# ParsaEsmati/SEA

Measured on AMD Instinct MI355X. Metric: rollout steps/sec (full-context forward, recompute mode) on cylinder_flow-shaped fields, higher is better.
Workload: dtype bf16

## Files before the change

### sea_amd/build.py

```python
from __future__ import annotations

import os
import subprocess
import sys
from concurrent.futures import ThreadPoolExecutor

HERE = os.path.dirname(os.path.abspath(__file__))
CSRC = os.path.join(HERE, "csrc")
BUILD = os.path.join(CSRC, "build")
LIB = os.path.join(CSRC, "libsea_hip.so")
SOURCES = ["core.hip", "gemm.hip", "gemm_norm.hip", "mlp_fused.hip", "attention.hip", "rowops.hip", "train.hip", "bwd.hip", "attention_bwd.hip", "kvstep.hip", "gemv.hip", "chain.hip", "gemm_adaln.hip", "mlp_block.hip", "adaln_qkv.hip", "gemm256.hip", "gemm_ws.hip", "encoder_block.hip", "decode_loss.hip", "ensemble.hip"]
HEADERS = ["sea_common.hpp", "gemm_core.hpp", "norm_epilogue.hpp", "gemm_tile.hpp", os.path.join("..", "..", "include", "sea_hip.h")]
FLAGS = (os.environ.get("SEA_EXTRA_FLAGS", "").split()) + ["--offload-arch=gfx950", "-O3", "-std=c++17", "-fPIC", "-mcode-object-version=5", "-mllvm", "-amdgpu-mfma-vgpr-form=1", "-ffast-math", "-fno-finite-math-only", "-fgpu-flush-denormals-to-zero", "-Wall", "-Wno-unused-function", "-Wno-unused-result"]


FILE_FLAGS: dict = {}

_PK_SRC1_HI = __import__("re").compile(r"^\s*v_pk_(?:fma|mul|add)_f32\b.*\bop_sel:\[[01],1[,\]]")


def lint_isa(asm_path: str) -> list:
    bad, kernel = [], "?"
    with open(asm_path) as f:
        for no, line in enumerate(f, 1):
            if line[:1].isalpha() or line[:1] == "_":
                kernel = line.split(":")[0]
            elif _PK_SRC1_HI.match(line):
                bad.append((kernel, no, line.strip()))
    return bad


def _hipcc() -> str:
    for cand in (os.environ.get("HIPCC"), "/opt/rocm/bin/hipcc", "hipcc"):
        if cand and (os.path.isabs(cand) and os.path.exists(cand) or not os.path.isabs(cand)):
            return cand
    raise RuntimeError("hipcc not found")


def _asm_of(obj: str) -> str:
    return obj[:-2] + "-hip-amdgcn-amd-amdhsa-gfx950.s"


def _stale(target: str, deps) -> bool:
    if not os.path.exists(target):
        return True
    t = os.path.getmtime(target)
    return any(os.path.getmtime(d) > t for d in deps if os.path.exists(d))


def build(force: bool = False, verbose: bool = True) -> str:
    import fcntl

    os.makedirs(BUILD, exist_ok=True)
    with open(os.path.join(CSRC, ".build.lock"), "w") as lock:
        fcntl.flock(lock, fcntl.LOCK_EX)
        try:
            return _build_locked(force, verbose)
        finally:
            fcntl.flock(lock, fcntl.LOCK_UN)


def _build_locked(force: bool, verbose: bool) -> str:
    hipcc = _hipcc()
    srcs = [s for s in SOURCES if os.path.exists(os.path.join(CSRC, s))]
    hdrs = [os.path.join(CSRC, h) for h in HEADERS]
    objs = []
    jobs = []
    os.makedirs(BUILD, exist_ok=True)
    for s in srcs:
        src = os.path.join(CSRC, s)
        obj = os.path.join(BUILD, s.replace(".hip", ".o"))
        objs.append(obj)
        if force or _stale(obj, [src] + hdrs) or not os.path.exists(_asm_of(obj)):
            jobs.append([hipcc] + FLAGS + FILE_FLAGS.get(s, []) + ["-save-temps=obj", "-c", src, "-o", obj])

    def run(cmd):
        if verbose:
            print(" ".join(cmd), flush=True)
        r = subprocess.run(cmd, stdout=subprocess.PIPE, stderr=subprocess.STDOUT, text=True)
        return r.returncode, r.stdout

    if jobs:
        with ThreadPoolExecutor(max_workers=min(4, len(jobs))) as ex:
            for rc, out in ex.map(run, jobs):
                if out.strip() and verbose:
                    print(out)
                if rc != 0:
                    raise RuntimeError("hipcc failed:\n" + out)
    for f in os.listdir(BUILD):
        stem = f.split("-hip-")[0].split(".")[0]
        if (not (f.endswith(".o") and "-hip-" not in f) and not f.endswith("-hip-amdgcn-amd-amdhsa-gfx950.s")) or stem + ".hip" not in srcs:
            try:
                os.remove(os.path.join(BUILD, f))
            except FileNotFoundError:
                pass
    findings = []
    for obj in objs:
        for kernel, no, ins in lint_isa(_asm_of(obj)):
            findings.append(f"{os.path.basename(_asm_of(obj))}:{no}: {kernel}: {ins}")
    if findings:
        for obj in objs:
            if lint_isa(_asm_of(obj)):
                os.remove(obj)
        raise RuntimeError("sea_amd.build: packed fp32 instructions with the low half reading the high dword of src1 (gfx950 erratum, see build.py):\n  "
                           + "\n  ".join(findings[:40]) + (f"\n  ... {len(findings) - 40} more" if len(findings) > 40 else ""))
    if force or jobs or _stale(LIB, objs):
        rc, out = run([hipcc, "--offload-arch=gfx950", "-shared", "-fPIC", "-o", LIB] + objs)
        if rc != 0:
            raise RuntimeError("link failed:\n" + out)
    return LIB


if __name__ == "__main__":
    print(build(force="--force" in sys.argv))
```

### sea_amd/csrc/mlp_block.hip

```cpp
#include "gemm_core.hpp"
#include <stdlib.h>

struct MlpBlockLaunch {
    SeaMlpGroup g1[SEA_MAX_MLP_GROUPS];
    SeaMlp2Group g2[SEA_MAX_MLP_GROUPS];
    int tile_start[SEA_MAX_MLP_GROUPS + 1];
    int xcd_start[SEA_MAX_MLP_GROUPS + 1];
    int n_groups;
    float eps;
    int per_xcd;
    int probe;
};

__device__ __forceinline__ void glds16_blk(const void* gsrc, unsigned lds_addr) {
    unsigned keep;
    asm volatile("s_mov_b32 %0, m0\n\ts_mov_b32 m0, %2\n\ts_nop 0\n\tglobal_load_lds_dwordx4 %1, off\n\ts_mov_b32 m0, %0"
                 : "=&s"(keep) : "v"(gsrc), "s"(lds_addr) : "memory");
}

__device__ __forceinline__ void glds16_blk_s(const void* ubase, unsigned lane_off, unsigned lds_addr) {
    unsigned keep;
    asm volatile("s_mov_b32 %0, m0\n\ts_mov_b32 m0, %3\n\ts_nop 0\n\tglobal_load_lds_dwordx4 %1, %2\n\ts_mov_b32 m0, %0"
                 : "=&s"(keep) : "v"(lane_off), "s"(ubase), "s"(lds_addr) : "memory");
}

template <int KT, int NSB>
struct MlpBlockCfg {
    static constexpr int BM = 32, BKB = 128, NS = 4, NW = 8;
    static constexpr int E = KT * 64, S = NSB * 128;
    static constexpr int A_BYTES = KT * BM * BKB, STAGE = KT * 64 * BKB;
    static constexpr int PRM_OFF = A_BYTES + NS * STAGE;
    static constexpr int P1_BYTES = PRM_OFF + 2 * S * 4;
    static constexpr int SLAB_PITCH = 128 * 4 + 16, SLAB = BM * SLAB_PITCH;
    static constexpr int X3_OFF = NW * SLAB;
    static constexpr int RED2_OFF = X3_OFF + KT * BM * BKB;
    static constexpr int P2_BYTES = RED2_OFF + 2 * NW * BM * 4;
    static constexpr int RS = KT == 4 ? 8 : 4, SLOT = 16 * 128;
    static constexpr int RING_OFF = KT == 4 ? A_BYTES : P1_BYTES;
    static constexpr int RING_END = RING_OFF + NW * RS * SLOT;
    static constexpr int BYTES_ = P1_BYTES > P2_BYTES ? P1_BYTES : P2_BYTES;
    static constexpr int BYTES = BYTES_ > RING_END ? BYTES_ : RING_END;
};

__device__ __forceinline__ f32x4 mma16_first(const uint4& a, const uint4& b) {
    return __builtin_amdgcn_mfma_f32_16x16x32_bf16(__builtin_bit_cast(bf16x8, a), __builtin_bit_cast(bf16x8, b), f32x4{0.f, 0.f, 0.f, 0.f}, 0, 0, 0);
}

__device__ __forceinline__ constexpr int blk_col_base(int t, int half, int wq) { return (t >> 1) * 512 + half * 256 + wq * 64 + (t & 1) * 32; }

template <int KT, int NSB>
__global__ __launch_bounds__(512) void mlp_block_kernel(const MlpBlockLaunch L) {
    using T = __bf16;
    using Cf = MlpBlockCfg<KT, NSB>;
    constexpr int BM = 32, BKB = 128, BK = 64, NS = 4, NW = 8;
    constexpr int E = Cf::E, S = Cf::S, NSTAGE = S / 64, NT = NSB / 2;
    constexpr int A_BYTES = Cf::A_BYTES, STAGE = Cf::STAGE;
    constexpr int LPS = KT * 8 / NW;
    constexpr int PRM_OFF = Cf::PRM_OFF;
    constexpr int B1_OFF = 0, RED_OFF = S * 4;
    static_assert(RED_OFF + 2 * NW * BM * 4 <= A_BYTES && (S / 256) * 1024 <= A_BYTES && LPS * NW == KT * 8 && NT % 2 == 0 && Cf::BYTES <= 160 * 1024, "LDS layout of sea_mlp_block");
    static_assert((NT / 2) * 512 == S, "blk_col_base covers the hidden columns once");
    extern __shared__ __attribute__((aligned(16))) char smem[];
    int tile, gi = 0;
    if (L.per_xcd < 0) {
        const int xcd = (int)(blockIdx.x & 7), idx = (int)(blockIdx.x >> 3);
        if (xcd >= L.xcd_start[L.n_groups]) return;
        while (gi + 1 < L.n_groups && xcd >= L.xcd_start[gi + 1]) ++gi;
        tile = L.tile_start[gi] + (xcd - L.xcd_start[gi]) * 32 + idx;
        if (tile >= L.tile_start[gi + 1]) return;
    } else {
        tile = L.per_xcd > 0 ? (int)(blockIdx.x & 7) * L.per_xcd + (int)(blockIdx.x >> 3) : (int)blockIdx.x;
        if (tile >= L.tile_start[L.n_groups]) return;
        while (gi + 1 < L.n_groups && tile >= L.tile_start[gi + 1]) ++gi;
    }
    const SeaMlpGroup& G = L.g1[gi];
    const SeaMlp2Group& H = L.g2[gi];
    const int m0 = (tile - L.tile_start[gi]) * BM, M = G.M;
    const int tid = threadIdx.x, lane = tid & 63;
    const int wave = __builtin_amdgcn_readfirstlane(tid >> 6);
    const int r = lane & 15, g = lane >> 4;
    const int half = wave >> 2, wq = wave & 3;
    const T* A = static_cast<const T*>(G.A);
    const T* W = static_cast<const T*>(G.W1);
    const unsigned lds_base = __builtin_amdgcn_readfirstlane((unsigned)(uintptr_t)smem);
    const int rl = lane >> 3;
    const int chunk = (lane & 7) ^ (rl & 7);
    for (int p = wave; p < 2 * (S / 256); p += NW) {
        const float* src = p < S / 256 ? G.lnw : G.lnb;
        const int q = p < S / 256 ? p : p - S / 256;
        glds16_blk(src + q * 256 + lane * 4, lds_base + (unsigned)(PRM_OFF + p * 1024));
    }
    for (int p = wave; G.X32 == nullptr && p < KT * (BM / 8); p += NW) {
        const int kt = p / (BM / 8), u = p - kt * (BM / 8);
        int row = m0 + u * 8 + rl;
        row = row < M ? row : M - 1;
        glds16_blk(A + (int64_t)row * G.lda + kt * BK + chunk * 8, lds_base + (unsigned)(kt * BM * BKB + u * 8 * BKB));
    }
    const unsigned w1_lane = (unsigned)(((8 * (rl >> 2) + (rl & 3)) * G.ldw + chunk * 8) * 2);
    auto dma_stage = [&](int s) {
        const unsigned base = lds_base + (unsigned)(A_BYTES + (s % NS) * STAGE);
        const int t = s >> 2, u = (s >> 1) & 1, hs = s & 1;
#pragma unroll
        for (int i = 0; i < LPS; ++i) {
            const int p = i * NW + wave;
            const int kt = p >> 3, u8 = p & 7;
            const int urow = blk_col_base(t, hs, u8 >> 1) + 16 * (u8 & 1) + 4 * u;
            glds16_blk_s(W + (int64_t)urow * G.ldw + kt * BK, w1_lane, base + (unsigned)(kt * 64 * BKB + u8 * 8 * BKB));
        }
    };
    dma_stage(0);
    if (G.X32 != nullptr) {
        constexpr int CPT = E / 16;
        const int prow = tid >> 4, pl = tid & 15;
        int row = m0 + prow;
        row = row < M ? row : M - 1;
        const int c0 = pl * CPT;
        float xv[CPT];
#pragma unroll
        for (int c = 0; c < CPT; c += 4) load4(G.X32 + (int64_t)row * G.ldx32 + c0 + c, *reinterpret_cast<float(*)[4]>(xv + c));
        if (G.addend != nullptr) {
#pragma unroll
            for (int c = 0; c < CPT; c += 4) {
                float av[4];
                load4(G.addend + (int64_t)row * G.ldadd + c0 + c, av);
#pragma unroll
                for (int e = 0; e < 4; ++e) xv[c + e] += av[e];
            }
        }
        float gq[CPT], bq[CPT];
#pragma unroll
        for (int c = 0; c < CPT; c += 4) {
            load4(G.gamma + c0 + c, *reinterpret_cast<float(*)[4]>(gq + c));
#pragma unroll
            for (int e = 0; e < 4; ++e) bq[c + e] = 0.f;
            if (G.beta != nullptr) load4(G.beta + c0 + c, *reinterpret_cast<float(*)[4]>(bq + c));
            if (G.mod != nullptr) {
                float mw[4], mb[4];
                const T* mod = static_cast<const T*>(G.mod) + (int64_t)row * G.ldmod;
                load4(mod + c0 + c, mw);
                load4(mod + E + c0 + c, mb);
#pragma unroll
                for (int e = 0; e < 4; ++e) {
                    gq[c + e] += 1.0f + mw[e];
                    bq[c + e] += mb[e];
                }
            }
        }
        float s4[4] = {0.f, 0.f, 0.f, 0.f};
#pragma unroll
        for (int c = 0; c < CPT; c += 4)
#pragma unroll
            for (int e = 0; e < 4; ++e) s4[e] = add1(s4[e], xv[c + e]);
        float sm_ = add1(add1(s4[0], s4[1]), add1(s4[2], s4[3]));
#pragma unroll
        for (int o = 8; o >= 1; o >>= 1) sm_ += __shfl_xor(sm_, o);
        const float mean = sm_ * (1.0f / (float)E);
        float q4[4] = {0.f, 0.f, 0.f, 0.f};
#pragma unroll
        for (int c = 0; c < CPT; c += 4)
#pragma unroll
            for (int e = 0; e < 4; ++e) {
                const float d_ = xv[c + e] - mean;
                q4[e] = fma1(d_, d_, q4[e]);
            }
        float sq = add1(add1(q4[0], q4[1]), add1(q4[2], q4[3]));
#pragma unroll
        for (int o = 8; o >= 1; o >>= 1) sq += __shfl_xor(sq, o);
        const float rstd = 1.0f / sqrtf(sq * (1.0f / (float)E) + G.norm_eps);
#pragma unroll
        for (int c = 0; c < CPT; c += 8) {
            const int col = c0 + c, kt = col >> 6, ck = (col & 63) >> 3;
            bf16x8 pv;
#pragma unroll
            for (int e = 0; e < 8; ++e) pv[e] = (__bf16)((xv[c + e] - mean) * rstd * gq[c + e] + bq[c + e]);
            *reinterpret_cast<bf16x8*>(smem + kt * BM * BKB + prow * BKB + ((ck ^ (prow & 7)) << 4)) = pv;
        }
        asm volatile("s_waitcnt vmcnt(0) lgkmcnt(0)" ::: "memory");
    }
    for (int s = 1; s < NS - 1; ++s) dma_stage(s);

    const T* W2 = static_cast<const T*>(H.W2);
    const unsigned w2_lane = (unsigned)((rl * H.ldw2 + chunk * 8) * 2);
    const T* Wp = static_cast<const T*>(H.Wproj);
    const unsigned wp_lane = (unsigned)((rl * H.ldwp + chunk * 8) * 2);
    constexpr int NSLOT = (E / 16) * (NT / 2);
    constexpr int NJ = E / NW / 16;
    constexpr int NX = NJ * KT;
    auto w2_slot = [&](int k) {
        const unsigned dst = lds_base + (unsigned)(Cf::RING_OFF + (wave * Cf::RS + (k % Cf::RS)) * Cf::SLOT);
        if (k < NSLOT) {
            const int tau = k / (E / 16), j = k - tau * (E / 16);
            const T* ub = W2 + (int64_t)(j * 16) * H.ldw2 + blk_col_base(2 * tau, half, wq);
#pragma unroll
            for (int u = 0; u < 2; ++u)
                glds16_blk_s(ub + (int64_t)(8 * u) * H.ldw2, w2_lane, dst + (unsigned)(u * 1024));
        } else {
            const int kk = k - NSLOT, j = kk / KT, kt = kk - j * KT;
            const T* ub = Wp + (int64_t)(wave * (E / NW) + j * 16) * H.ldwp + kt * BK;
#pragma unroll
            for (int u = 0; u < 2; ++u)
                glds16_blk_s(ub + (int64_t)(8 * u) * H.ldwp, wp_lane, dst + (unsigned)(u * 1024));
        }
    };
    uint4 hid[NT][2];
    float mean[2], rstd[2];
    {
        f32x4 acc[NSB][2];
        uint4 areg[KT][2][2];
#pragma unroll
        for (int i = 0; i < NSB; ++i) {
            acc[i][0] = f32x4{0.f, 0.f, 0.f, 0.f};
            acc[i][1] = f32x4{0.f, 0.f, 0.f, 0.f};
        }
#pragma unroll
        for (int s = 0; s < NSTAGE; ++s) {
            if (s + 2 < NSTAGE) asm volatile("s_waitcnt vmcnt(%0) lgkmcnt(0)" ::"n"(2 * LPS) : "memory");
            else if (s + 1 < NSTAGE) asm volatile("s_waitcnt vmcnt(%0) lgkmcnt(0)" ::"n"(LPS) : "memory");
            else asm volatile("s_waitcnt vmcnt(0) lgkmcnt(0)" ::: "memory");
            __builtin_amdgcn_s_barrier();
            if (s + NS - 1 < NSTAGE) dma_stage(s + NS - 1);
            if (s == 0) {
                const char* sA = smem + r * BKB;
#pragma unroll
                for (int kt = 0; kt < KT; ++kt)
#pragma unroll
                    for (int kc = 0; kc < 2; ++kc) {
                        const int off = ((kc * 4 + g) ^ (r & 7)) << 4;
                        areg[kt][kc][0] = *reinterpret_cast<const uint4*>(sA + kt * BM * BKB + off);
                        areg[kt][kc][1] = *reinterpret_cast<const uint4*>(sA + kt * BM * BKB + 16 * BKB + off);
                    }
                asm volatile("s_waitcnt lgkmcnt(0)" ::: "memory");
            }
            if (s == 1)
                for (int p = wave; p < S / 256; p += NW) glds16_blk(G.b1 + p * 256 + lane * 4, lds_base + (unsigned)(B1_OFF + p * 1024));
            if ((s & 1) == half) {
                const char* sW = smem + A_BYTES + (s % NS) * STAGE + (wq * 16 + r) * BKB;
#pragma unroll
                for (int kt = 0; kt < KT; ++kt)
#pragma unroll
                    for (int kc = 0; kc < 2; ++kc) {
                        const int off = ((kc * 4 + g) ^ (r & 7)) << 4;
                        const uint4 wf = *reinterpret_cast<const uint4*>(sW + kt * 64 * BKB + off);
                        mma16<T>(wf, areg[kt][kc][0], acc[s >> 1][0]);
                        mma16<T>(wf, areg[kt][kc][1], acc[s >> 1][1]);
                    }
            }
        }
        if (L.probe == 1) return;
        float* red = reinterpret_cast<float*>(smem + RED_OFF);
        const float* pb1 = reinterpret_cast<const float*>(smem + B1_OFF);
        const float* pgm = reinterpret_cast<const float*>(smem + PRM_OFF);
        const float* pbt = pgm + S;
        const float inv_s = 1.0f / (float)S;
        float sum[2] = {0.f, 0.f};
#pragma unroll
        for (int i = 0; i < NSB; ++i) {
            const int n = blk_col_base(i >> 1, half, wq) + 8 * g + 4 * (i & 1);
            float bv[4];
            load4(pb1 + n, bv);
#pragma unroll
            for (int mb = 0; mb < 2; ++mb) {
#pragma unroll
                for (int q = 0; q < 4; ++q) acc[i][mb][q] += bv[q];
                sum[mb] += (acc[i][mb][0] + acc[i][mb][1]) + (acc[i][mb][2] + acc[i][mb][3]);
            }
        }
#pragma unroll
        for (int mb = 0; mb < 2; ++mb) {
            sum[mb] += __shfl_xor(sum[mb], 16);
            sum[mb] += __shfl_xor(sum[mb], 32);
            if (g == 0) red[wave * 32 + mb * 16 + r] = sum[mb];
        }
        __syncthreads();
#pragma unroll
        for (int k = 0; k < Cf::RS - 1; ++k) w2_slot(k);
        float sq[2] = {0.f, 0.f};
#pragma unroll
        for (int mb = 0; mb < 2; ++mb) {
            float t = 0.f;
#pragma unroll
            for (int w = 0; w < NW; ++w) t += red[w * 32 + mb * 16 + r];
            mean[mb] = t * inv_s;
        }
#pragma unroll
        for (int i = 0; i < NSB; ++i)
#pragma unroll
            for (int mb = 0; mb < 2; ++mb)
#pragma unroll
                for (int q = 0; q < 4; ++q) {
                    const float c = acc[i][mb][q] - mean[mb];
                    sq[mb] += c * c;
                }
#pragma unroll
        for (int mb = 0; mb < 2; ++mb) {
            sq[mb] += __shfl_xor(sq[mb], 16);
            sq[mb] += __shfl_xor(sq[mb], 32);
            if (g == 0) red[256 + wave * 32 + mb * 16 + r] = sq[mb];
        }
        asm volatile("s_waitcnt lgkmcnt(0)" ::: "memory");
        __builtin_amdgcn_s_barrier();
#pragma unroll
        for (int mb = 0; mb < 2; ++mb) {
            float t = 0.f;
#pragma unroll
            for (int w = 0; w < NW; ++w) t += red[256 + w * 32 + mb * 16 + r];
            rstd[mb] = 1.0f / sqrtf(t * inv_s + L.eps);
        }
#pragma unroll
        for (int i = 0; i < NSB; ++i) {
            const int n = blk_col_base(i >> 1, half, wq) + 8 * g + 4 * (i & 1);
            float gm[4], bt[4];
            load4(pgm + n, gm);
            load4(pbt + n, bt);
#pragma unroll
            for (int mb = 0; mb < 2; ++mb) {
                bf16x4 y;
#pragma unroll
                for (int q = 0; q < 4; ++q) y[q] = (__bf16)gelu_erf_bf16((acc[i][mb][q] - mean[mb]) * rstd[mb] * gm[q] + bt[q]);
                uint2 y2 = *reinterpret_cast<const uint2*>(&y);
                asm volatile("" : "+v"(y2.x), "+v"(y2.y));
                if (i & 1) {
                    hid[i >> 1][mb].z = y2.x;
                    hid[i >> 1][mb].w = y2.y;
                } else {
                    hid[i >> 1][mb].x = y2.x;
                    hid[i >> 1][mb].y = y2.y;
                }
            }
            __builtin_amdgcn_sched_barrier(0);
        }
    }
    __builtin_amdgcn_sched_barrier(0);
    if (L.probe == 2) {
        asm volatile("s_waitcnt vmcnt(0)" ::: "memory");
        return;
    }

    constexpr int NJB = E / 16;
    constexpr int NTOT = NSLOT + NX;
    f32x4 acc2[2][NJB];
    uint4 wp[KT * 2][NJ];
#pragma unroll
    for (int k = 0; k < NTOT; ++k) {
        const int tau = k / NJB, j = k - tau * NJB;
        {
            constexpr int AFTER_MAX = Cf::RS - 2;
            const int after = NTOT - 1 - k < AFTER_MAX ? NTOT - 1 - k : AFTER_MAX;
            switch (after) {
                case 6: asm volatile("s_waitcnt vmcnt(12) lgkmcnt(0)" ::: "memory"); break;
                case 5: asm volatile("s_waitcnt vmcnt(10) lgkmcnt(0)" ::: "memory"); break;
                case 4: asm volatile("s_waitcnt vmcnt(8) lgkmcnt(0)" ::: "memory"); break;
                case 3: asm volatile("s_waitcnt vmcnt(6) lgkmcnt(0)" ::: "memory"); break;
                case 2: asm volatile("s_waitcnt vmcnt(4) lgkmcnt(0)" ::: "memory"); break;
                case 1: asm volatile("s_waitcnt vmcnt(2) lgkmcnt(0)" ::: "memory"); break;
                default: asm volatile("s_waitcnt vmcnt(0) lgkmcnt(0)" ::: "memory"); break;
            }
        }
        if (k + Cf::RS - 1 < NTOT) w2_slot(k + Cf::RS - 1);
        const char* sl = smem + Cf::RING_OFF + (wave * Cf::RS + (k % Cf::RS)) * Cf::SLOT + r * 128;
        if (k >= NSLOT) {
            const int kk = k - NSLOT, jp = kk / KT, kt = kk - jp * KT;
#pragma unroll
            for (int kc = 0; kc < 2; ++kc) wp[kt * 2 + kc][jp] = *reinterpret_cast<const uint4*>(sl + (((kc * 4 + g) ^ (r & 7)) << 4));
            continue;
        }
#pragma unroll
        for (int u2 = 0; u2 < 2; ++u2) {
            const uint4 w = *reinterpret_cast<const uint4*>(sl + (((u2 * 4 + g) ^ (r & 7)) << 4));
            const int t = 2 * tau + u2;
            if (t == 0) {
                acc2[0][j] = mma16_first(w, hid[0][0]);
                acc2[1][j] = mma16_first(w, hid[0][1]);
            } else {
                mma16<T>(w, hid[t][0], acc2[0][j]);
                mma16<T>(w, hid[t][1], acc2[1][j]);
            }
        }
        __builtin_amdgcn_sched_barrier(0);
    }
    __syncthreads();
    if (L.probe == 3) return;
    {
    int tid_l = threadIdx.x;
    asm volatile("" : "+v"(tid_l));
    const int tid = tid_l, lane = tid & 63, r = lane & 15, g = lane >> 4;
    (void)lane;
    constexpr int NH = E / 128, JH = 8;
    const int srow = tid >> 4, scb = (tid & 15) * 8;
    float resv[NH][8];
    {
        int row = m0 + srow;
        row = row < M ? row : M - 1;
#pragma unroll
        for (int h = 0; h < NH; ++h) {
            const int col = h * 128 + scb;
            float b2a[4], b2b[4];
            load4(H.b2 + col, b2a);
            load4(H.b2 + col + 4, b2b);
            float ra[4], rb[4];
            if (H.R != nullptr) {
                load4(H.R + (int64_t)row * H.ldr + col, ra);
                load4(H.R + (int64_t)row * H.ldr + col + 4, rb);
            } else {
                load4(G.X32 + (int64_t)row * G.ldx32 + col, ra);
                load4(G.X32 + (int64_t)row * G.ldx32 + col + 4, rb);
                if (G.addend != nullptr) {
                    float aa[4], ab[4];
                    load4(G.addend + (int64_t)row * G.ldadd + col, aa);
                    load4(G.addend + (int64_t)row * G.ldadd + col + 4, ab);
#pragma unroll
                    for (int q = 0; q < 4; ++q) {
                        ra[q] += aa[q];
                        rb[q] += ab[q];
                    }
                }
            }
#pragma unroll
            for (int q = 0; q < 4; ++q) {
                resv[h][q] = b2a[q] + ra[q];
                resv[h][4 + q] = b2b[q] + rb[q];
            }
        }
    }
    constexpr int CPT = E / 16;
    const int ec0 = (tid & 15) * CPT;
    float ebp[CPT], egq[CPT], ebq[CPT];
    const bool has_norm = H.gamma != nullptr;
#pragma unroll
    for (int h = 0; h < NH; ++h) {
        char* slab = smem + wave * Cf::SLAB;
#pragma unroll
        for (int mb = 0; mb < 2; ++mb)
#pragma unroll
            for (int j = 0; j < JH; ++j)
                *reinterpret_cast<f32x4*>(slab + (mb * 16 + r) * Cf::SLAB_PITCH + (j * 16 + g * 4) * 4) = acc2[mb][h * JH + j];
        if (h == NH - 1) {
            __builtin_amdgcn_sched_barrier(0);
            int m = m0 + srow;
            m = m < M ? m : M - 1;
#pragma unroll
            for (int c = 0; c < CPT; c += 4) {
                load4(H.bproj + ec0 + c, *reinterpret_cast<float(*)[4]>(ebp + c));
#pragma unroll
                for (int q = 0; q < 4; ++q) egq[c + q] = ebq[c + q] = 0.f;
                if (has_norm) {
                    load4(H.gamma + ec0 + c, *reinterpret_cast<float(*)[4]>(egq + c));
                    if (H.beta != nullptr) load4(H.beta + ec0 + c, *reinterpret_cast<float(*)[4]>(ebq + c));
                    if (H.mod != nullptr) {
                        float mw[4], mb[4];
                        const T* mod = static_cast<const T*>(H.mod) + (int64_t)m * H.ldmod;
                        load4(mod + ec0 + c, mw);
                        load4(mod + E + ec0 + c, mb);
#pragma unroll
                        for (int q = 0; q < 4; ++q) {
                            egq[c + q] += 1.0f + mw[q];
                            ebq[c + q] += mb[q];
                        }
                    }
                }
            }
        }
        asm volatile("s_waitcnt lgkmcnt(0)" ::: "memory");
        __builtin_amdgcn_s_barrier();
        {
            float v[8];
#pragma unroll
            for (int q = 0; q < 8; ++q) v[q] = resv[h][q];
#pragma unroll
            for (int w = 0; w < NW; ++w) {
                const float4 a = *reinterpret_cast<const float4*>(smem + w * Cf::SLAB + srow * Cf::SLAB_PITCH + scb * 4);
                const float4 b = *reinterpret_cast<const float4*>(smem + w * Cf::SLAB + srow * Cf::SLAB_PITCH + scb * 4 + 16);
                v[0] += a.x; v[1] += a.y; v[2] += a.z; v[3] += a.w;
                v[4] += b.x; v[5] += b.y; v[6] += b.z; v[7] += b.w;
            }
            const int col = h * 128 + scb, kt = col >> 6, ck = (col & 63) >> 3;
            bf16x8 pv;
#pragma unroll
            for (int q = 0; q < 8; ++q) pv[q] = (__bf16)v[q];
            *reinterpret_cast<bf16x8*>(smem + Cf::X3_OFF + kt * BM * BKB + srow * BKB + ((ck ^ (srow & 7)) << 4)) = pv;
        }
        asm volatile("s_waitcnt lgkmcnt(0)" ::: "memory");
        __builtin_amdgcn_s_barrier();
        if (L.probe == 5 + h) return;
    }

    if (L.probe == 4) return;
    f32x4 acc3[2][NJ];
    {
        const char* sA = smem + Cf::X3_OFF + r * BKB;
#pragma unroll
        for (int kt = 0; kt < KT; ++kt)
#pragma unroll
            for (int kc = 0; kc < 2; ++kc) {
                const int off = ((kc * 4 + g) ^ (r & 7)) << 4;
                const uint4 af0 = *reinterpret_cast<const uint4*>(sA + kt * BM * BKB + off);
                const uint4 af1 = *reinterpret_cast<const uint4*>(sA + kt * BM * BKB + 16 * BKB + off);
#pragma unroll
                for (int j = 0; j < NJ; ++j) {
                    if (kt == 0 && kc == 0) {
                        acc3[0][j] = mma16_first(wp[0][j], af0);
                        acc3[1][j] = mma16_first(wp[0][j], af1);
                    } else {
                        mma16<T>(wp[kt * 2 + kc][j], af0, acc3[0][j]);
                        mma16<T>(wp[kt * 2 + kc][j], af1, acc3[1][j]);
                    }
                }
            }
    }
    constexpr int SEG = 80, YP = (E / 16) * SEG + 16;
    static_assert(BM * YP <= Cf::X3_OFF, "the y tile lies in front of the x3 tile");
#pragma unroll
    for (int i = 0; i < 2; ++i)
#pragma unroll
        for (int j = 0; j < NJ; ++j) {
            const int n = wave * (E / NW) + j * 16 + g * 4;
            *reinterpret_cast<f32x4*>(smem + (i * 16 + r) * YP + (n >> 4) * SEG + (n & 15) * 4) = acc3[i][j];
        }
    asm volatile("s_waitcnt lgkmcnt(0)" ::: "memory");
    __builtin_amdgcn_s_barrier();
    {
        float v[CPT];
#pragma unroll
        for (int c = 0; c < CPT; c += 4) {
            const float4 y = *reinterpret_cast<const float4*>(smem + srow * YP + ((ec0 + c) >> 4) * SEG + ((ec0 + c) & 15) * 4);
            v[c] = y.x + ebp[c]; v[c + 1] = y.y + ebp[c + 1]; v[c + 2] = y.z + ebp[c + 2]; v[c + 3] = y.w + ebp[c + 3];
        }
        if (has_norm) {
            float s4[4] = {0.f, 0.f, 0.f, 0.f};
#pragma unroll
            for (int c = 0; c < CPT; c += 4)
#pragma unroll
                for (int e = 0; e < 4; ++e) s4[e] = add1(s4[e], v[c + e]);
            float sm_ = add1(add1(s4[0], s4[1]), add1(s4[2], s4[3]));
#pragma unroll
            for (int o = 8; o >= 1; o >>= 1) sm_ += __shfl_xor(sm_, o);
            const float mean2 = sm_ * (1.0f / (float)E);
            float q4[4] = {0.f, 0.f, 0.f, 0.f};
#pragma unroll
            for (int c = 0; c < CPT; c += 4)
#pragma unroll
                for (int e = 0; e < 4; ++e) {
                    const float d_ = v[c + e] - mean2;
                    q4[e] = fma1(d_, d_, q4[e]);
                }
            float sq = add1(add1(q4[0], q4[1]), add1(q4[2], q4[3]));
#pragma unroll
            for (int o = 8; o >= 1; o >>= 1) sq += __shfl_xor(sq, o);
            const float rstd2 = 1.0f / sqrtf(sq * (1.0f / (float)E) + L.eps);
#pragma unroll
            for (int c = 0; c < CPT; ++c) v[c] = (v[c] - mean2) * rstd2 * egq[c] + ebq[c];
        }
        const int m = m0 + srow;
        if (m < M) {
#pragma unroll
            for (int c = 0; c < CPT; c += 4) {
                if (H.Y32 != nullptr) store4(H.Y32 + (int64_t)m * H.ldy32 + ec0 + c, v[c], v[c + 1], v[c + 2], v[c + 3]);
                if (H.Yact != nullptr) store4(static_cast<T*>(H.Yact) + (int64_t)m * H.ldyact + ec0 + c, v[c], v[c + 1], v[c + 2], v[c + 3]);
            }
        }
    }
    }
}

extern "C" int sea_mlp_block(const SeaMlpGroup* g1, const SeaMlp2Group* g2, int n_groups, float eps, int dtype, void* stream) {
    SEA_REQUIRE(g1 != nullptr && g2 != nullptr && n_groups >= 1 && n_groups <= SEA_MAX_MLP_GROUPS, "sea_mlp_block: n_groups=%d out of range", n_groups);
    const int E = g1[0].E, S = g1[0].S;
    const bool shape_ok = (E == 256 && S == 2048) || (E == 128 && S == 1024);
    if (dtype != SEA_BF16 || !shape_ok) {
        sea_set_error("sea_mlp_block: unsupported dtype / shape (dtype=%d E=%d S=%d): bf16, (E, S) in {(256, 2048), (128, 1024)}", dtype, E, S);
        return SEA_EUNSUPPORTED;
    }
    MlpBlockLaunch L;
    memset(&L, 0, sizeof(L));
    int total = 0;
    for (int i = 0; i < n_groups; ++i) {
        const SeaMlpGroup& G = g1[i];
        const SeaMlp2Group& H = g2[i];
        SEA_REQUIRE(G.E == E && G.S == S && H.E == E && H.S == S && G.M >= 1 && H.M == G.M, "sea_mlp_block[%d]: the groups of a launch share E and S; both halves the same M", i);
        SEA_REQUIRE((G.A || G.X32) && G.W1 && G.b1 && G.lnw && G.lnb, "sea_mlp_block[%d]: null pointer (first layer)", i);
        SEA_REQUIRE((G.X32 || (G.lda % 8 == 0 && G.lda >= E)) && G.ldw % 8 == 0 && G.ldw >= E, "sea_mlp_block[%d]: bad strides (first layer)", i);
        if (G.X32 != nullptr)
            SEA_REQUIRE(G.gamma && G.ldx32 % 4 == 0 && G.ldx32 >= E && (!G.addend || (G.ldadd % 4 == 0 && G.ldadd >= E)) && G.Xout == nullptr &&
                            (!G.mod || (G.ldmod % 8 == 0 && G.ldmod >= 2 * E)) && sea_aligned16(G.X32) && sea_aligned16(G.addend) && sea_aligned16(G.mod) &&
                            sea_aligned16(G.gamma) && sea_aligned16(G.beta) && G.norm_eps > 0.f,
                        "sea_mlp_block[%d]: norm prologue: null / misaligned pointer, bad stride, or Xout (the block keeps x + addend to itself)", i);
        SEA_REQUIRE(sea_aligned16(G.A) && sea_aligned16(G.W1) && sea_aligned16(G.b1) && sea_aligned16(G.lnw) && sea_aligned16(G.lnb), "sea_mlp_block[%d]: pointers must be 16-byte aligned", i);
        SEA_REQUIRE(H.W2 && H.b2 && (H.R || G.X32) && H.Wproj && H.bproj && (H.Y32 || H.Yact), "sea_mlp_block[%d]: null pointer (second layer; R may be NULL with the norm prologue: the residual is then x + addend)", i);
        SEA_REQUIRE(H.ldw2 % 8 == 0 && H.ldw2 >= S && H.ldwp % 8 == 0 && H.ldwp >= E && (!H.R || (H.ldr % 4 == 0 && H.ldr >= E)) &&
                        (!H.Y32 || (H.ldy32 % 4 == 0 && H.ldy32 >= E)) && (!H.Yact || (H.ldyact % 4 == 0 && H.ldyact >= E)) && (!H.mod || (H.ldmod % 4 == 0 && H.ldmod >= 2 * E)),
                    "sea_mlp_block[%d]: bad strides (second layer)", i);
        SEA_REQUIRE(sea_aligned16(H.W2) && sea_aligned16(H.b2) && sea_aligned16(H.R) && sea_aligned16(H.Wproj) && sea_aligned16(H.bproj) && sea_aligned16(H.gamma) && sea_aligned16(H.beta) &&
                        sea_aligned16(H.mod) && sea_aligned16(H.Y32) && sea_aligned16(H.Yact),
                    "sea_mlp_block[%d]: pointers must be 16-byte aligned", i);
        SEA_REQUIRE(H.gamma || (!H.beta && !H.mod), "sea_mlp_block[%d]: beta / mod without gamma", i);
        L.g1[i] = G;
        L.g2[i] = H;
        L.tile_start[i] = total;
        total += (G.M + 31) / 32;
    }
    L.tile_start[n_groups] = total;
    L.n_groups = n_groups;
    L.eps = eps;
    static const int probe = sea_tune("blk_probe", 0);
    L.probe = probe;
    hipStream_t s = static_cast<hipStream_t>(stream);
    int xcds = 0;
    for (int i = 0; i < n_groups; ++i) {
        L.xcd_start[i] = xcds;
        xcds += (L.tile_start[i + 1] - L.tile_start[i] + 31) / 32;
    }
    L.xcd_start[n_groups] = xcds;
    static const int xcd_excl = sea_tune("blk_xcd", 0);
    static const int per_xcd_on = sea_tune("blk_perxcd", 1);
    if (total > 256 && per_xcd_on) {
        L.per_xcd = (total + 7) / 8;
        total = 8 * L.per_xcd;
    } else if (xcds <= 8 && xcd_excl) {
        L.per_xcd = -1;
        total = 256;
    }
    if (E == 256) {
        constexpr int lds = MlpBlockCfg<4, 16>::BYTES;
        static const hipError_t once = hipFuncSetAttribute(reinterpret_cast<const void*>(mlp_block_kernel<4, 16>), hipFuncAttributeMaxDynamicSharedMemorySize, lds);
        (void)once;
        mlp_block_kernel<4, 16><<<dim3(total), dim3(512), lds, s>>>(L);
    } else {
        constexpr int lds = MlpBlockCfg<2, 8>::BYTES;
        static const hipError_t once = hipFuncSetAttribute(reinterpret_cast<const void*>(mlp_block_kernel<2, 8>), hipFuncAttributeMaxDynamicSharedMemorySize, lds);
        (void)once;
        mlp_block_kernel<2, 8><<<dim3(total), dim3(512), lds, s>>>(L);
    }
    SEA_CHECK_LAUNCH("sea_mlp_block");
    return SEA_OK;
}
```

Measured before the change: 5189.

## Stream W1 through a per-wave private LDS ring in the E=256 MLP block

For E=256, the W1 GEMM phase now has each wave prefetch its own W1 slices into a private 8-slot LDS ring using global_load_lds and fine-grained vmcnt waits. This replaces the shared 4-stage dma_stage pipeline and its block-wide barriers. The LN prologue and epilogue loads for addend, beta and mod are also hoisted and batched ahead of their arithmetic, so more memory latency overlaps. The new path is on by default through a tune knob. It depends on hand-counted waitcnt values, which risk correctness if the per-wave load counts drift.

```diff
diff --git a/sea_amd/build.py b/sea_amd/build.py
--- a/sea_amd/build.py
+++ b/sea_amd/build.py
@@ -10,7 +10,7 @@
 BUILD = os.path.join(CSRC, "build")
 LIB = os.path.join(CSRC, "libsea_hip.so")
 SOURCES = ["core.hip", "gemm.hip", "gemm_norm.hip", "mlp_fused.hip", "attention.hip", "rowops.hip", "train.hip", "bwd.hip", "attention_bwd.hip", "kvstep.hip", "gemv.hip", "chain.hip", "gemm_adaln.hip", "mlp_block.hip", "adaln_qkv.hip", "gemm256.hip", "gemm_ws.hip", "encoder_block.hip", "decode_loss.hip", "ensemble.hip"]
-HEADERS = ["sea_common.hpp", "gemm_core.hpp", "norm_epilogue.hpp", "gemm_tile.hpp", os.path.join("..", "..", "include", "sea_hip.h")]
+HEADERS = ["sea_common.hpp", "gemm_core.hpp", "norm_epilogue.hpp", "gemm_tile.hpp", "mlp_block_ring.hpp", os.path.join("..", "..", "include", "sea_hip.h")]
 FLAGS = (os.environ.get("SEA_EXTRA_FLAGS", "").split()) + ["--offload-arch=gfx950", "-O3", "-std=c++17", "-fPIC", "-mcode-object-version=5", "-mllvm", "-amdgpu-mfma-vgpr-form=1", "-ffast-math", "-fno-finite-math-only", "-fgpu-flush-denormals-to-zero", "-Wall", "-Wno-unused-function", "-Wno-unused-result"]
 
 
diff --git a/sea_amd/csrc/mlp_block.hip b/sea_amd/csrc/mlp_block.hip
--- a/sea_amd/csrc/mlp_block.hip
+++ b/sea_amd/csrc/mlp_block.hip
@@ -1,4 +1,5 @@
 #include "gemm_core.hpp"
+#include "mlp_block_ring.hpp"
 #include <stdlib.h>
 
 struct MlpBlockLaunch {
@@ -38,6 +39,8 @@
     static constexpr int RS = KT == 4 ? 8 : 4, SLOT = 16 * 128;
     static constexpr int RING_OFF = KT == 4 ? A_BYTES : P1_BYTES;
     static constexpr int RING_END = RING_OFF + NW * RS * SLOT;
+    static constexpr int RS1 = 8, RING1_OFF = A_BYTES;
+    static_assert(KT != 4 || (RING1_OFF + NW * RS1 * SLOT == PRM_OFF && RING1_OFF == RING_OFF && RS1 == RS), "the W1 ring fills the shared ring's region");
     static constexpr int BYTES_ = P1_BYTES > P2_BYTES ? P1_BYTES : P2_BYTES;
     static constexpr int BYTES = BYTES_ > RING_END ? BYTES_ : RING_END;
 };
@@ -46,9 +49,21 @@
     return __builtin_amdgcn_mfma_f32_16x16x32_bf16(__builtin_bit_cast(bf16x8, a), __builtin_bit_cast(bf16x8, b), f32x4{0.f, 0.f, 0.f, 0.f}, 0, 0, 0);
 }
 
-__device__ __forceinline__ constexpr int blk_col_base(int t, int half, int wq) { return (t >> 1) * 512 + half * 256 + wq * 64 + (t & 1) * 32; }
-
-template <int KT, int NSB>
+
+__device__ __forceinline__ void blk_w1_wait(int pieces) {
+    switch (pieces) {
+        case 13: asm volatile("s_waitcnt vmcnt(13) lgkmcnt(0)" ::: "memory"); break;
+        case 12: asm volatile("s_waitcnt vmcnt(12) lgkmcnt(0)" ::: "memory"); break;
+        case 10: asm volatile("s_waitcnt vmcnt(10) lgkmcnt(0)" ::: "memory"); break;
+        case 8: asm volatile("s_waitcnt vmcnt(8) lgkmcnt(0)" ::: "memory"); break;
+        case 6: asm volatile("s_waitcnt vmcnt(6) lgkmcnt(0)" ::: "memory"); break;
+        case 4: asm volatile("s_waitcnt vmcnt(4) lgkmcnt(0)" ::: "memory"); break;
+        case 2: asm volatile("s_waitcnt vmcnt(2) lgkmcnt(0)" ::: "memory"); break;
+        default: asm volatile("s_waitcnt vmcnt(0) lgkmcnt(0)" ::: "memory"); break;
+    }
+}
+
+template <int KT, int NSB, bool RING1>
 __global__ __launch_bounds__(512) void mlp_block_kernel(const MlpBlockLaunch L) {
     using T = __bf16;
     using Cf = MlpBlockCfg<KT, NSB>;
@@ -60,6 +75,7 @@
     constexpr int B1_OFF = 0, RED_OFF = S * 4;
     static_assert(RED_OFF + 2 * NW * BM * 4 <= A_BYTES && (S / 256) * 1024 <= A_BYTES && LPS * NW == KT * 8 && NT % 2 == 0 && Cf::BYTES <= 160 * 1024, "LDS layout of sea_mlp_block");
     static_assert((NT / 2) * 512 == S, "blk_col_base covers the hidden columns once");
+    static_assert(!RING1 || (KT == 4 && S / 256 == NW && KT * (BM / 8) == 2 * NW), "private W1 ring: E = 256, S = 2048 (every wave issues the same number of lnw | lnb, A and b1 pieces: its waits count them)");
     extern __shared__ __attribute__((aligned(16))) char smem[];
     int tile, gi = 0;
     if (L.per_xcd < 0) {
@@ -108,42 +124,65 @@
             glds16_blk_s(W + (int64_t)urow * G.ldw + kt * BK, w1_lane, base + (unsigned)(kt * 64 * BKB + u8 * 8 * BKB));
         }
     };
-    dma_stage(0);
+    auto w1_slot = [&](int k) {
+        const BlkW1Slot sl = blk_w1_slot<KT, Cf::RS1>(wave, k);
+        const T* ub = W + (int64_t)sl.row0 * G.ldw + sl.kt * BK;
+        const unsigned dst = lds_base + (unsigned)(Cf::RING1_OFF + sl.lds);
+#pragma unroll
+        for (int u = 0; u < 2; ++u)
+            glds16_blk_s(ub + (int64_t)(16 * u) * G.ldw, w1_lane, dst + (unsigned)(u * BLK_PIECE_BYTES));
+    };
+    if constexpr (RING1) {
+#pragma unroll
+        for (int k = 0; k < Cf::RS1 - 1; ++k) w1_slot(k);
+    } else {
+        dma_stage(0);
+    }
     if (G.X32 != nullptr) {
         constexpr int CPT = E / 16;
         const int prow = tid >> 4, pl = tid & 15;
         int row = m0 + prow;
         row = row < M ? row : M - 1;
         const int c0 = pl * CPT;
-        float xv[CPT];
+        float xv[CPT], av[CPT], gq[CPT], bq[CPT], mw[CPT], mb[CPT];
+        const bool has_add = G.addend != nullptr, has_mod = G.mod != nullptr;
 #pragma unroll
         for (int c = 0; c < CPT; c += 4) load4(G.X32 + (int64_t)row * G.ldx32 + c0 + c, *reinterpret_cast<float(*)[4]>(xv + c));
-        if (G.addend != nullptr) {
-#pragma unroll
-            for (int c = 0; c < CPT; c += 4) {
-                float av[4];
-                load4(G.addend + (int64_t)row * G.ldadd + c0 + c, av);
-#pragma unroll
-                for (int e = 0; e < 4; ++e) xv[c + e] += av[e];
-            }
-        }
-        float gq[CPT], bq[CPT];
+        if (has_add) {
+#pragma unroll
+            for (int c = 0; c < CPT; c += 4) load4(G.addend + (int64_t)row * G.ldadd + c0 + c, *reinterpret_cast<float(*)[4]>(av + c));
+        }
 #pragma unroll
         for (int c = 0; c < CPT; c += 4) {
             load4(G.gamma + c0 + c, *reinterpret_cast<float(*)[4]>(gq + c));
 #pragma unroll
             for (int e = 0; e < 4; ++e) bq[c + e] = 0.f;
-            if (G.beta != nullptr) load4(G.beta + c0 + c, *reinterpret_cast<float(*)[4]>(bq + c));
-            if (G.mod != nullptr) {
-                float mw[4], mb[4];
-                const T* mod = static_cast<const T*>(G.mod) + (int64_t)row * G.ldmod;
-                load4(mod + c0 + c, mw);
-                load4(mod + E + c0 + c, mb);
-#pragma unroll
-                for (int e = 0; e < 4; ++e) {
-                    gq[c + e] += 1.0f + mw[e];
-                    bq[c + e] += mb[e];
-                }
+        }
+        if (G.beta != nullptr) {
+#pragma unroll
+            for (int c = 0; c < CPT; c += 4) load4(G.beta + c0 + c, *reinterpret_cast<float(*)[4]>(bq + c));
+        }
+        if (has_mod) {
+            const T* mod = static_cast<const T*>(G.mod) + (int64_t)row * G.ldmod;
+#pragma unroll
+            for (int c = 0; c < CPT; c += 4) {
+                load4(mod + c0 + c, *reinterpret_cast<float(*)[4]>(mw + c));
+                load4(mod + E + c0 + c, *reinterpret_cast<float(*)[4]>(mb + c));
+            }
+        }
+        if (has_add) {
+#pragma unroll
+            for (int c = 0; c < CPT; ++c) {
+                xv[c] += av[c];
+                asm volatile("" : "+v"(xv[c]));
+            }
+        }
+        if (has_mod) {
+#pragma unroll
+            for (int c = 0; c < CPT; ++c) {
+                gq[c] += 1.0f + mw[c];
+                bq[c] += mb[c];
+                asm volatile("" : "+v"(gq[c]), "+v"(bq[c]));
             }
         }
         float s4[4] = {0.f, 0.f, 0.f, 0.f};
@@ -177,7 +216,8 @@
         }
         asm volatile("s_waitcnt vmcnt(0) lgkmcnt(0)" ::: "memory");
     }
-    for (int s = 1; s < NS - 1; ++s) dma_stage(s);
+    if constexpr (!RING1)
+        for (int s = 1; s < NS - 1; ++s) dma_stage(s);
 
     const T* W2 = static_cast<const T*>(H.W2);
     const unsigned w2_lane = (unsigned)((rl * H.ldw2 + chunk * 8) * 2);
@@ -212,6 +252,45 @@
             acc[i][0] = f32x4{0.f, 0.f, 0.f, 0.f};
             acc[i][1] = f32x4{0.f, 0.f, 0.f, 0.f};
         }
+        if constexpr (RING1) {
+            asm volatile("s_waitcnt vmcnt(%0) lgkmcnt(0)" ::"n"(2 * (Cf::RS1 - 1)) : "memory");
+            __builtin_amdgcn_s_barrier();
+            {
+                const char* sA = smem + r * BKB;
+#pragma unroll
+                for (int kt = 0; kt < KT; ++kt)
+#pragma unroll
+                    for (int kc = 0; kc < 2; ++kc) {
+                        const int off = ((kc * 4 + g) ^ (r & 7)) << 4;
+                        areg[kt][kc][0] = *reinterpret_cast<const uint4*>(sA + kt * BM * BKB + off);
+                        areg[kt][kc][1] = *reinterpret_cast<const uint4*>(sA + kt * BM * BKB + 16 * BKB + off);
+                    }
+                asm volatile("s_waitcnt lgkmcnt(0)" ::: "memory");
+            }
+            __builtin_amdgcn_s_barrier();
+            if (L.probe == 9) {
+                asm volatile("s_waitcnt vmcnt(0)" ::: "memory");
+                return;
+            }
+            glds16_blk(G.b1 + wave * 256 + lane * 4, lds_base + (unsigned)(B1_OFF + wave * 1024));
+            constexpr int NK = blk_w1_slots<KT, NSB>();
+#pragma unroll
+            for (int k = 0; k < NK; ++k) {
+                const int after = NK - 1 - k < Cf::RS1 - 2 ? NK - 1 - k : Cf::RS1 - 2;
+                blk_w1_wait(2 * after + (k < Cf::RS1 - 1 ? 1 : 0));
+                if (k + Cf::RS1 - 1 < NK) w1_slot(k + Cf::RS1 - 1);
+                const int i = k / KT, kt = k - i * KT;
+                const char* sl = smem + Cf::RING1_OFF + (wave * Cf::RS1 + (k % Cf::RS1)) * Cf::SLOT + r * 128;
+#pragma unroll
+                for (int kc = 0; kc < 2; ++kc) {
+                    const uint4 wf = *reinterpret_cast<const uint4*>(sl + (((kc * 4 + g) ^ (r & 7)) << 4));
+                    mma16<T>(wf, areg[kt][kc][0], acc[i][0]);
+                    mma16<T>(wf, areg[kt][kc][1], acc[i][1]);
+                }
+                __builtin_amdgcn_sched_barrier(0);
+            }
+            __builtin_amdgcn_s_barrier();
+        } else {
 #pragma unroll
         for (int s = 0; s < NSTAGE; ++s) {
             if (s + 2 < NSTAGE) asm volatile("s_waitcnt vmcnt(%0) lgkmcnt(0)" ::"n"(2 * LPS) : "memory");
@@ -245,6 +324,7 @@
                         mma16<T>(wf, areg[kt][kc][1], acc[s >> 1][1]);
                     }
             }
+        }
         }
         if (L.probe == 1) return;
         float* red = reinterpret_cast<float*>(smem + RED_OFF);
@@ -425,7 +505,8 @@
     constexpr int CPT = E / 16;
     const int ec0 = (tid & 15) * CPT;
     float ebp[CPT], egq[CPT], ebq[CPT];
-    const bool has_norm = H.gamma != nullptr;
+    float emw[CPT], emb[CPT];
+    const bool has_norm = H.gamma != nullptr, has_emod = has_norm && H.mod != nullptr;
 #pragma unroll
     for (int h = 0; h < NH; ++h) {
         char* slab = smem + wave * Cf::SLAB;
@@ -443,20 +524,21 @@
                 load4(H.bproj + ec0 + c, *reinterpret_cast<float(*)[4]>(ebp + c));
 #pragma unroll
                 for (int q = 0; q < 4; ++q) egq[c + q] = ebq[c + q] = 0.f;
-                if (has_norm) {
-                    load4(H.gamma + ec0 + c, *reinterpret_cast<float(*)[4]>(egq + c));
-                    if (H.beta != nullptr) load4(H.beta + ec0 + c, *reinterpret_cast<float(*)[4]>(ebq + c));
-                    if (H.mod != nullptr) {
-                        float mw[4], mb[4];
-                        const T* mod = static_cast<const T*>(H.mod) + (int64_t)m * H.ldmod;
-                        load4(mod + ec0 + c, mw);
-                        load4(mod + E + ec0 + c, mb);
-#pragma unroll
-                        for (int q = 0; q < 4; ++q) {
-                            egq[c + q] += 1.0f + mw[q];
-                            ebq[c + q] += mb[q];
-                        }
-                    }
+            }
+            if (has_norm) {
+#pragma unroll
+                for (int c = 0; c < CPT; c += 4) load4(H.gamma + ec0 + c, *reinterpret_cast<float(*)[4]>(egq + c));
+            }
+            if (has_norm && H.beta != nullptr) {
+#pragma unroll
+                for (int c = 0; c < CPT; c += 4) load4(H.beta + ec0 + c, *reinterpret_cast<float(*)[4]>(ebq + c));
+            }
+            if (has_emod) {
+                const T* mod = static_cast<const T*>(H.mod) + (int64_t)m * H.ldmod;
+#pragma unroll
+                for (int c = 0; c < CPT; c += 4) {
+                    load4(mod + ec0 + c, *reinterpret_cast<float(*)[4]>(emw + c));
+                    load4(mod + E + ec0 + c, *reinterpret_cast<float(*)[4]>(emb + c));
                 }
             }
         }
@@ -547,6 +629,14 @@
 #pragma unroll
             for (int o = 8; o >= 1; o >>= 1) sq += __shfl_xor(sq, o);
             const float rstd2 = 1.0f / sqrtf(sq * (1.0f / (float)E) + L.eps);
+            if (has_emod) {
+#pragma unroll
+                for (int c = 0; c < CPT; ++c) {
+                    egq[c] += 1.0f + emw[c];
+                    ebq[c] += emb[c];
+                    asm volatile("" : "+v"(egq[c]), "+v"(ebq[c]));
+                }
+            }
 #pragma unroll
             for (int c = 0; c < CPT; ++c) v[c] = (v[c] - mean2) * rstd2 * egq[c] + ebq[c];
         }
@@ -619,17 +709,24 @@
         L.per_xcd = -1;
         total = 256;
     }
-    if (E == 256) {
+    const bool ring1 = E == 256 && sea_tune("blk_ring1", 1) != 0;
+    if (E == 256 && ring1) {
         constexpr int lds = MlpBlockCfg<4, 16>::BYTES;
-        static const hipError_t once = hipFuncSetAttribute(reinterpret_cast<const void*>(mlp_block_kernel<4, 16>), hipFuncAttributeMaxDynamicSharedMemorySize, lds);
+        static const hipError_t once = hipFuncSetAttribute(reinterpret_cast<const void*>(mlp_block_kernel<4, 16, true>), hipFuncAttributeMaxDynamicSharedMemorySize, lds);
         (void)once;
-        mlp_block_kernel<4, 16><<<dim3(total), dim3(512), lds, s>>>(L);
+        mlp_block_kernel<4, 16, true><<<dim3(total), dim3(512), lds, s>>>(L);
+    } else if (E == 256) {
+        constexpr int lds = MlpBlockCfg<4, 16>::BYTES;
+        static const hipError_t once = hipFuncSetAttribute(reinterpret_cast<const void*>(mlp_block_kernel<4, 16, false>), hipFuncAttributeMaxDynamicSharedMemorySize, lds);
+        (void)once;
+        mlp_block_kernel<4, 16, false><<<dim3(total), dim3(512), lds, s>>>(L);
     } else {
         constexpr int lds = MlpBlockCfg<2, 8>::BYTES;
-        static const hipError_t once = hipFuncSetAttribute(reinterpret_cast<const void*>(mlp_block_kernel<2, 8>), hipFuncAttributeMaxDynamicSharedMemorySize, lds);
+        static const hipError_t once = hipFuncSetAttribute(reinterpret_cast<const void*>(mlp_block_kernel<2, 8, false>), hipFuncAttributeMaxDynamicSharedMemorySize, lds);
         (void)once;
-        mlp_block_kernel<2, 8><<<dim3(total), dim3(512), lds, s>>>(L);
+        mlp_block_kernel<2, 8, false><<<dim3(total), dim3(512), lds, s>>>(L);
     }
     SEA_CHECK_LAUNCH("sea_mlp_block");
+    sea_note_form(ring1 ? "mlp_block.ring" : "mlp_block.stage", 0, 0);
     return SEA_OK;
 }
diff --git a/sea_amd/csrc/mlp_block_ring.hpp b/sea_amd/csrc/mlp_block_ring.hpp
--- /dev/null
+++ b/sea_amd/csrc/mlp_block_ring.hpp
@@ -0,0 +1,28 @@
+#pragma once
+
+#if defined(__HIPCC__) || defined(__CUDACC__)
+#define SEA_RING_HD __host__ __device__ __forceinline__
+#else
+#define SEA_RING_HD inline
+#endif
+
+SEA_RING_HD constexpr int blk_col_base(int t, int half, int wq) { return (t >> 1) * 512 + half * 256 + wq * 64 + (t & 1) * 32; }
+
+struct BlkW1Slot {
+    int row0;
+    int kt;
+    int lds;
+};
+
+constexpr int BLK_SLOT_BYTES = 16 * 128, BLK_PIECE_BYTES = 8 * 128, BLK_WAVES = 8;
+
+SEA_RING_HD constexpr int blk_w1_row_of(int m) { return 8 * (m >> 2) + (m & 3); }
+
+template <int KT, int NSB>
+SEA_RING_HD constexpr int blk_w1_slots() { return NSB * KT; }
+
+template <int KT, int RS>
+SEA_RING_HD constexpr BlkW1Slot blk_w1_slot(int wave, int k) {
+    const int i = k / KT, kt = k - i * KT;
+    return BlkW1Slot{blk_col_base(i >> 1, wave >> 2, wave & 3) + 4 * (i & 1), kt, (wave * RS + k % RS) * BLK_SLOT_BYTES};
+}
```

Result: no change. 5239, median of 4 (+1.0%).
